# ubc-vision/DiffuseSG

Hardware: NVIDIA B200
Metric: sampled scene graphs/sec (higher is better)
Workload: dtype bf16

## Files before the change

diffusesg_b200/csrc/blockhead.cu:

```cuda
#include <cstdlib>

#include "common.cuh"
#include "kernels.h"

namespace dsg {
namespace {

constexpr int kHeadThreads = 19 * 32;
constexpr float kHeadLnEps = 1e-5f;

template <int C>
struct HeadCfg {
  static constexpr int N3 = 3 * C;
  static constexpr int KBN = C / 32;
  static constexpr int W_KB = C * 64;
  static constexpr int W_BYTES = 3 * KBN * W_KB;
  static constexpr int XB = C / 32;
  static constexpr int X_BYTES = XB * 16384;
  static constexpr int QB = C / 32;
  static constexpr int Q_BYTES = QB * 8192;
  static constexpr int CW = C / 4;
  static constexpr int PAR_FLOATS = N3 + 2 * C;
  static constexpr int PART_BYTES = 4 * 128 * 4;
  static constexpr int SMEM_BYTES = 1024 + W_BYTES + 2 * X_BYTES + 2 * Q_BYTES + PART_BYTES + PAR_FLOATS * 4 + 256;
  static constexpr int Y_COL = 3 * C;
  static_assert(C % 32 == 0 && CW % 8 == 0, "head: C must be a multiple of 32");
  static_assert(Y_COL + C / 2 <= 512 && SMEM_BYTES <= 227 * 1024, "head budget");
};

struct HeadParams {
  const float* film;
  int film_ld;
  int cond_uniform;
  int tokens_per_sample;
  const float* gamma;
  const float* beta;
  const float* bqkv;
  int M;
};

DSG_DEVICE uint64_t umma_desc_sw64_h(uint32_t smem_addr) {
  const uint64_t lo = ((smem_addr & 0x3FFFFu) >> 4) | (1ull << 16);
  const uint64_t hi = (512u >> 4) | (1u << 14) | (4u << 29);
  return lo | (hi << 32);
}
DSG_DEVICE void umma_bf16_ts_h(uint32_t tmem_d, uint32_t tmem_a, uint64_t b_desc, uint32_t idesc, uint32_t accumulate) {
  asm volatile(
      "{\n\t"
      ".reg .pred p;\n\t"
      "setp.ne.b32 p, %4, 0;\n\t"
      "tcgen05.mma.cta_group::1.kind::f16 [%0], [%1], %2, %3, p;\n\t"
      "}"
      ::"r"(tmem_d), "r"(tmem_a), "l"(b_desc), "r"(idesc), "r"(accumulate)
      : "memory");
}
DSG_DEVICE void tmem_ld_32x8_h(uint32_t taddr, uint32_t* r) {
  asm volatile("tcgen05.ld.sync.aligned.32x32b.x8.b32 {%0, %1, %2, %3, %4, %5, %6, %7}, [%8];"
               : "=r"(r[0]), "=r"(r[1]), "=r"(r[2]), "=r"(r[3]), "=r"(r[4]), "=r"(r[5]), "=r"(r[6]), "=r"(r[7])
               : "r"(taddr)
               : "memory");
}
DSG_DEVICE void tmem_st_32x4_h(uint32_t taddr, const uint32_t* r) {
  asm volatile("tcgen05.st.sync.aligned.32x32b.x4.b32 [%0], {%1, %2, %3, %4};"
               ::"r"(taddr), "r"(r[0]), "r"(r[1]), "r"(r[2]), "r"(r[3])
               : "memory");
}
DSG_DEVICE void tmem_st_wait_h() { asm volatile("tcgen05.wait::st.sync.aligned;" ::: "memory"); }
DSG_DEVICE void tma_store_2d_h(const CUtensorMap* map, const void* smem_src, int c_inner, int c_outer) {
  asm volatile("cp.async.bulk.tensor.2d.global.shared::cta.bulk_group [%0, {%2, %3}], [%1];"
               ::"l"(reinterpret_cast<uint64_t>(map)), "r"(smem_u32(smem_src)), "r"(c_inner), "r"(c_outer)
               : "memory");
}

template <int C>
__global__ void __launch_bounds__(kHeadThreads, 1)
block_head_kernel(const __grid_constant__ CUtensorMap tmXin, const __grid_constant__ CUtensorMap tmXout,
                  const __grid_constant__ CUtensorMap tmW, const __grid_constant__ CUtensorMap tmQ, const HeadParams p) {
  using G = HeadCfg<C>;
  extern __shared__ uint8_t smem_raw[];
  uint8_t* smem = smem_raw + ((1024u - (smem_u32(smem_raw) & 1023u)) & 1023u);
  uint8_t* sW = smem;
  uint8_t* sX = sW + G::W_BYTES;
  uint8_t* sXo = sX + G::X_BYTES;
  uint8_t* sQ = sXo + G::X_BYTES;
  float* sPart = reinterpret_cast<float*>(sQ + 2 * G::Q_BYTES);
  float* sBq = reinterpret_cast<float*>(reinterpret_cast<uint8_t*>(sPart) + G::PART_BYTES);
  float* sGam = sBq + G::N3;
  float* sBet = sGam + C;
  uint64_t* bars = reinterpret_cast<uint64_t*>(sBet + C);
  uint64_t* w_full = bars;
  uint64_t* xin_full = bars + 1;
  uint64_t* xin_free = bars + 2;
  uint64_t* xo_ready = bars + 3;
  uint64_t* xo_free = bars + 4;
  uint64_t* y_ready = bars + 5;
  uint64_t* acc_full = bars + 6;
  uint64_t* acc_empty = bars + 7;
  uint64_t* q_ready = bars + 8;
  uint64_t* q_free = bars + 10;
  uint32_t* tmem_slot = reinterpret_cast<uint32_t*>(bars + 12);

  const int warp = uniform_warp_id();
  const int lane = threadIdx.x & 31;
  constexpr int kLoadWarp = 16, kMmaWarp = 17, kStoreWarp = 18;
  const int num_tiles = (p.M + 127) / 128;
  const int my_tiles = (num_tiles > static_cast<int>(blockIdx.x)) ? (num_tiles - blockIdx.x + gridDim.x - 1) / gridDim.x : 0;

  if (warp == kLoadWarp && lane == 0) {
    tma_prefetch_desc(&tmXin);
    tma_prefetch_desc(&tmXout);
    tma_prefetch_desc(&tmW);
    tma_prefetch_desc(&tmQ);
    mbar_init(w_full, 1);
    mbar_init(xin_full, 1);
    mbar_init(xin_free, 16);
    mbar_init(xo_ready, 16);
    mbar_init(xo_free, 1);
    mbar_init(y_ready, 16);
    mbar_init(acc_full, 1);
    mbar_init(acc_empty, 16);
    for (int b = 0; b < 2; ++b) { mbar_init(&q_ready[b], 16); mbar_init(&q_free[b], 1); }
    fence_barrier_init();
  }
  if (warp == kMmaWarp) tmem_alloc<512>(tmem_slot);
  for (int i = threadIdx.x; i < G::N3; i += kHeadThreads) sBq[i] = p.bqkv[i];
  for (int i = threadIdx.x; i < C; i += kHeadThreads) { sGam[i] = p.gamma[i]; sBet[i] = p.beta[i]; }
  tcgen05_fence_before();
  __syncthreads();
  tcgen05_fence_after();
  const uint32_t tmem_base = uniform_u32(*tmem_slot);

  if (warp == kLoadWarp) {
    if (elect_one()) {
      mbar_expect_tx(w_full, G::W_BYTES);
      for (int part = 0; part < 3; ++part)
        for (int kb = 0; kb < G::KBN; ++kb)
          tma_load_2d(sW + (part * G::KBN + kb) * G::W_KB, &tmW, w_full, kb * 32, part * C);
      auto load_x = [&](int tl) {
        const int tile = blockIdx.x + tl * gridDim.x;
        mbar_expect_tx(xin_full, G::X_BYTES);
        for (int xb = 0; xb < G::XB; ++xb) tma_load_2d(sX + xb * 16384, &tmXin, xin_full, xb * 32, tile * 128);
      };
      auto prefetch_x = [&](int tl) {
        const int tile = blockIdx.x + tl * gridDim.x;
        for (int xb = 0; xb < G::XB; ++xb)
          asm volatile("cp.async.bulk.prefetch.tensor.2d.L2.global.tile [%0, {%1, %2}];"
                       ::"l"(reinterpret_cast<uint64_t>(&tmXin)), "r"(xb * 32), "r"(tile * 128) : "memory");
// ... 101 lines not shown
      asm volatile("bar.sync 1, 512;" ::: "memory");
      const float mean = ((sPart[r_t] + sPart[128 + r_t]) + (sPart[256 + r_t] + sPart[384 + r_t])) * (1.0f / C);
      float qq = 0.f;
#pragma unroll
      for (int i = 0; i < G::CW; i += 4) {
        float4& x = v[i >> 2];
        x.x -= mean; x.y -= mean; x.z -= mean; x.w -= mean;
        qq += (x.x * x.x + x.y * x.y) + (x.z * x.z + x.w * x.w);
      }
      asm volatile("bar.sync 2, 512;" ::: "memory");
      sPart[cg * 128 + r_t] = qq;
      asm volatile("bar.sync 1, 512;" ::: "memory");
      const float rstd =
          rsqrtf(((sPart[r_t] + sPart[128 + r_t]) + (sPart[256 + r_t] + sPart[384 + r_t])) * (1.0f / C) + kHeadLnEps);
      if (tl > 0) mbar_wait(acc_full, (tl - 1) & 1);
      tcgen05_fence_after();
#pragma unroll
      for (int i = 0; i < G::CW; i += 8) {
        const float4 g0 = *reinterpret_cast<const float4*>(&sGam[c0 + i]), g1 = *reinterpret_cast<const float4*>(&sGam[c0 + i + 4]);
        const float4 b0 = *reinterpret_cast<const float4*>(&sBet[c0 + i]), b1 = *reinterpret_cast<const float4*>(&sBet[c0 + i + 4]);
        const float4 xa = v[i >> 2], xb = v[(i >> 2) + 1];
        uint32_t pk[4];
        pk[0] = pack_bf16x2(fmaf(xa.x * rstd, g0.x, b0.x), fmaf(xa.y * rstd, g0.y, b0.y));
        pk[1] = pack_bf16x2(fmaf(xa.z * rstd, g0.z, b0.z), fmaf(xa.w * rstd, g0.w, b0.w));
        pk[2] = pack_bf16x2(fmaf(xb.x * rstd, g1.x, b1.x), fmaf(xb.y * rstd, g1.y, b1.y));
        pk[3] = pack_bf16x2(fmaf(xb.z * rstd, g1.z, b1.z), fmaf(xb.w * rstd, g1.w, b1.w));
        tmem_st_32x4_h(t_lane + G::Y_COL + ((c0 + i) >> 1), pk);
      }
      tmem_st_wait_h();
      tcgen05_fence_before();
      __syncwarp();
      if (lane == 0) mbar_arrive(y_ready);
    };

    int k = 0;
    auto phase_e = [&](int tl) {
      mbar_wait(acc_full, tl & 1);
      tcgen05_fence_after();
#pragma unroll 1
      for (int part = 0; part < 3; ++part, ++k) {
        const int b = k & 1;
        uint32_t v[G::CW];
#pragma unroll
        for (int i = 0; i < G::CW; i += 8) tmem_ld_32x8_h(t_lane + part * C + c0 + i, v + i);
        tmem_ld_wait();
        if (part == 2) {
          tcgen05_fence_before();
          __syncwarp();
          if (lane == 0) mbar_arrive(acc_empty);
        }
        if (k >= 2) mbar_wait(&q_free[b], ((k >> 1) - 1) & 1);
        uint8_t* buf = sQ + b * G::Q_BYTES;
#pragma unroll
        for (int i = 0; i < G::CW; i += 8) {
          const int c = c0 + i;
          const float4 ba = *reinterpret_cast<const float4*>(&sBq[part * C + c]);
          const float4 bb = *reinterpret_cast<const float4*>(&sBq[part * C + c + 4]);
          uint4 w;
          w.x = pack_bf16x2(__uint_as_float(v[i]) + ba.x, __uint_as_float(v[i + 1]) + ba.y);
          w.y = pack_bf16x2(__uint_as_float(v[i + 2]) + ba.z, __uint_as_float(v[i + 3]) + ba.w);
          w.z = pack_bf16x2(__uint_as_float(v[i + 4]) + bb.x, __uint_as_float(v[i + 5]) + bb.y);
          w.w = pack_bf16x2(__uint_as_float(v[i + 6]) + bb.z, __uint_as_float(v[i + 7]) + bb.w);
          *reinterpret_cast<uint4*>(buf + (c >> 5) * 8192 + r_t * 64 + (((((c & 31) >> 3)) ^ ((r_t >> 1) & 3)) << 4)) = w;
        }
        fence_proxy_async_smem();
        __syncwarp();
        if (lane == 0) mbar_arrive(&q_ready[b]);
      }
    };

    if (my_tiles > 0) phase_f(0);
    for (int tl = 0; tl < my_tiles; ++tl) {
      if (tl + 1 < my_tiles) phase_f(tl + 1);
      phase_e(tl);
    }
  }

  tcgen05_fence_before();
  __syncthreads();
  tcgen05_fence_after();
  if (warp == kMmaWarp) tmem_dealloc<512>(tmem_base);
}

}

bool block_head_supported(int C) { return C == 96; }

int launch_block_head(const CUtensorMap* tmXin, const CUtensorMap* tmXout, const CUtensorMap* tmW, const CUtensorMap* tmQ,
                      const float* film, int film_ld, int cond_uniform, int tokens_per_sample, const float* gamma,
                      const float* beta, const float* bqkv, long long rows, int C, cudaStream_t st) {
  DSG_REQUIRE(block_head_supported(C) && rows > 0 && rows < 2147483647LL, "block_head: C=%d rows=%lld", C, rows);
  using G = HeadCfg<96>;
  static PerDeviceOnce configured;
  if (configured.first()) {
    DSG_CUDA_CHECK(cudaFuncSetAttribute(block_head_kernel<96>, cudaFuncAttributeMaxDynamicSharedMemorySize, G::SMEM_BYTES));
  }
  const int sms = device_sm_count();
  HeadParams p{film, film_ld, cond_uniform, tokens_per_sample, gamma, beta, bqkv, static_cast<int>(rows)};
  const int tiles = (p.M + 127) / 128;
  block_head_kernel<96><<<tiles < sms ? tiles : sms, kHeadThreads, G::SMEM_BYTES, st>>>(*tmXin, *tmXout, *tmW, *tmQ, p);
  DSG_LAUNCH_CHECK();
  return DSG_OK;
}

}
```

diffusesg_b200/csrc/kernels.h:

```cpp
#pragma once

#include <cuda.h>
#include <cuda_bf16.h>
#include <cuda_runtime.h>
#include <stdint.h>

namespace dsg {

typedef __nv_bfloat16 bf16;

enum GemmEpi : int {
  EPI_BF16 = 0,
  EPI_GELU_BF16 = 1,
  EPI_RES_F32 = 2,
  EPI_F32 = 3,
  EPI_ADJ_HEAD = 4,
};

struct GemmParams {
  int M, N, K;
  const float* bias;
  const float* res;
  void* out;
  int ldo;
  int bn;
  int ksplit;
  int scale_rows;
  float row_scale;
  const float* w2t;
  const float* b2;
  int c_e;
  int n_img;
  const uint8_t* flags;
  const float* x_adj;
  const float* c_skip;
  const float* c_out;
  const int* perm;
  int side;
};

int make_tmap_bf16(CUtensorMap* map, const void* base, int64_t rows, int64_t cols, int box_rows);
int make_tmap_out(CUtensorMap* map, const void* base, int64_t rows, int64_t cols, int epi);

int launch_wgrad(const void* dy, const void* x, float* dw, long long tokens, int n_out, int x_cols, int out_cols, int ksplit,
                 int scale_rows, float row_scale, cudaStream_t st);

int gemm_block_n(int N);
int gemm_choose_bn(long long rows, int N, int K, int epi, bool pair);
bool gemm_use_pair(long long rows, int K, int epi);
int launch_gemm(const CUtensorMap* tmA, const CUtensorMap* tmW, const CUtensorMap* tmO, int epi, const GemmParams& p,
                cudaStream_t st, bool pair = false);

bool fused_mlp_supported(int C);
int fused_mlp_w1_box_rows(int C);
int launch_fused_mlp(const CUtensorMap* tmY, const CUtensorMap* tmW1, const CUtensorMap* tmW2, const CUtensorMap* tmX,
                     const float* b1, const float* b2, long long rows, int C, cudaStream_t st);

int make_tmap_2d(CUtensorMap* map, const void* base, int64_t rows, int64_t cols, int elem_bytes, int box_cols,
                 int box_rows);
bool block_tail_supported(int C);
int launch_block_tail(const CUtensorMap* tmAtt, const CUtensorMap* tmWp, const CUtensorMap* tmW1,
                      const CUtensorMap* tmW2, const CUtensorMap* tmX, const float* bp, const float* gamma,
                      const float* beta, const float* b1, const float* b2, float* x, long long rows, int C,
                      cudaStream_t st, const CUtensorMap* tmY = nullptr,
                      const float* gamma_f = nullptr, const float* beta_f = nullptr);

bool proj_ln_supported(int C);
int launch_proj_ln(const CUtensorMap* tmA, const CUtensorMap* tmW, const float* bias, const float* gamma, const float* beta,
                   float* x, bf16* y, long long rows, int C, cudaStream_t st);

bool block_head_supported(int C);
int launch_block_head(const CUtensorMap* tmXin, const CUtensorMap* tmXout, const CUtensorMap* tmW, const CUtensorMap* tmQ,
                      const float* film, int film_ld, int cond_uniform, int tokens_per_sample, const float* gamma,
                      const float* beta, const float* bqkv, long long rows, int C, cudaStream_t st);

int make_tmap_3d_bf16(CUtensorMap* map, const void* base, int64_t d0, int64_t d1, int64_t d2, int64_t s1, int64_t s2, int b0,
                      int b1, int b2);
bool window_attention_tc_supported(int batch, int res, int window, int shift, int heads);
int launch_window_attention_tc(const bf16* qkv, const float* bias, bf16* out, int batch, int res, int shift, int heads,
                               cudaStream_t st);
int launch_window_attention_tc_groups(const bf16* qkv, const float* bias, bf16* out, int n_groups, const int* counts,
                                      const int* res, const long long* tok_off, int heads, cudaStream_t st);
bool window_attention_quad_supported(int batch, int res, int window, int shift, int heads);
int launch_window_attention_quad(const bf16* qkv, const float* bias, bf16* out, int batch, int res, int window, int shift,
                                 int heads, cudaStream_t st);
int check_mask_canonical(const float* mask, int res, int window, int shift, cudaStream_t st, int* canonical);
bool window_attention_w16_supported(int batch, int res, int window, int shift, int heads);
int launch_window_attention_w16(const bf16* qkv, const float* bias, bf16* out, int batch, int res, int shift, int heads,
                                cudaStream_t st);
int check_bias_toeplitz(const float* bias, int heads, int window, cudaStream_t st, int* toeplitz);
enum { ATTN_MASK_CANONICAL = 1, ATTN_BIAS_TOEPLITZ = 2 };
int launch_window_attention(const bf16* qkv, const float* bias, const float* mask, bf16* out, int batch, int res,
                            int window, int shift, int heads, cudaStream_t st, int canonical = 0);

int launch_film_ln(const float* x_in, float* x_out, bf16* y, const float* film, int film_ld, int film_off,
                   int cond_uniform, const float* gamma, const float* beta, int batch, int tokens_per_sample,
                   int C, cudaStream_t st, const int* src_rows = nullptr);
int launch_ln(const float* x, bf16* y, const float* gamma, const float* beta, int64_t rows, int C, cudaStream_t st);
int launch_merge_ln(const float* x, bf16* y, const float* gamma, const float* beta, int batch, int res, int C,
                    cudaStream_t st);
int launch_concat_bf16(const float* x, const float* skip, bf16* y, int64_t rows, int C, cudaStream_t st,
                       const int* skip_rows = nullptr);
int launch_breakup_ln(const float* t, bf16* y, const float* g1, const float* b1, const float* g2, const float* b2,
                      int batch, int res, int D, cudaStream_t st, const int* tok0 = nullptr, const int* width = nullptr,
                      int sh = 0, const int* src_perm = nullptr);

int launch_cond(const float* noise_labels, long long label_stride, int n_cond, const float* w0, const float* b0, const float* w1,
                const float* b1, const float* w_film, const float* b_film, int film_total, float* emb0, float* emb1,
                float* emb, float* film, int embed, cudaStream_t st);

int launch_precond_coef(const float* sigmas, int sigma_stride, float* coef, int batch, cudaStream_t st);

int launch_node_proj(const float* node, const float* sc_node, const float* in_scale, const float* w_rc,
                     float* rc, int batch, int n, int c_n, int self_cond, int embed, cudaStream_t st);
int launch_patch_embed(const float* adj, const float* sc_adj, const float* in_scale, const uint8_t* flags,
                       const float* rc, const float* w_adj, const float* bias, const float* gamma,
                       const float* beta, const float* film, int film_ld, int film_off, int cond_uniform,
                       float* x0, int batch, int n, int c_e, int self_cond, int embed, cudaStream_t st,
                       const int* perm = nullptr, int side = 0);
int launch_node_head(const bf16* rep, const uint8_t* flags, const float* fold_t, const float* fold_b, const float* w1t,
                     const float* b1, const float* w2t, const float* b2, const float* x_node, const float* c_skip, const float* c_out,
                     float* out_node, int batch, int n, int c_n, int embed, cudaStream_t st, const int* tok0 = nullptr,
                     const int* width = nullptr, float* scratch = nullptr);


int launch_edm_pre_step(const float* adj, const float* node, const float* eps_adj, const float* eps_node,
                        const uint8_t* flags, float noise_coef, float* adj_hat, float* node_hat, int batch,
                        int c_e, int n, int c_n, cudaStream_t st);
int launch_edm_pre_step_philox(const float* adj, const float* node, const uint8_t* flags, float noise_coef,
                               unsigned long long seed, unsigned long long offset_adj, int grid_adj,
                               unsigned long long offset_node, int grid_node, const void* dev_params, float* adj_hat,
                               float* node_hat, int batch, int c_e, int n, int c_n, cudaStream_t st);
int launch_edm_post_step(const float* adj_hat, const float* node_hat, const float* d1_adj, const float* d1_node,
                         const float* d2_adj, const float* d2_node, const uint8_t* flags, float inv_t_hat,
                         float h, float inv_t_prime, const void* dev_params, float* adj_next, float* node_next, int batch,
                         int c_e, int n, int c_n, cudaStream_t st);
int launch_edm_step_advance(const void* table, void* cur, int* counter, cudaStream_t st);
int launch_edm_final_decode(const float* adj_hat, const float* node_hat, const float* d1_adj, const float* d1_node,
                            const uint8_t* flags, float inv_t_hat, float h, const void* dev_params, float* adj_next,
                            float* node_next, int32_t* adj_cls, int32_t* node_cls, float* bbox, int num_adj_type,
                            int num_node_type, int batch, int c_e, int n, int c_n, cudaStream_t st);
int launch_mask_scale(const float* adj, const float* node, const uint8_t* flags, float scale, float* adj_out,
                      float* node_out, int batch, int c_e, int n, int c_n, cudaStream_t st);

int launch_decode(const float* adj, const float* node, const uint8_t* flags, int32_t* adj_cls, int32_t* node_cls,
                  float* bbox, int num_adj_type, int num_node_type, int batch, int c_e, int n, int c_n, cudaStream_t st);

int launch_train_noise(const float* y_adj, const float* y_node, const float* e_adj, const float* e_node,
                       const float* sigmas, const uint8_t* flags, float* x_adj, float* n_adj, float* x_node,
                       float* n_node, int batch, int c_e, int n, int c_n, cudaStream_t st);
int launch_loss_sums(const float* d_adj, const float* y_adj, const float* d_node, const float* y_node,
                     const float* weights, const uint8_t* flags, float* s_adj, float* s_node, int batch, int c_e, int n,
                     int c_n, cudaStream_t st);
int launch_loss_sums_backward(const float* d_adj, const float* y_adj, const float* d_node, const float* y_node,
                              const float* weights, const uint8_t* flags, const float* g_adj, const float* g_node,
                              float* gd_adj, float* gd_node, int batch, int c_e, int n, int c_n, cudaStream_t st);

// ... 12 lines not shown
```

diffusesg_b200/csrc/model.cu:

```cuda
#include <cstdarg>
#include <cstdio>
#include <cstdlib>
#include <cstring>
#include <map>
#include <string>
#include <tuple>
#include <vector>

#include "../../include/dsg_b200.h"
#include "common.cuh"
#include "kernels.h"

namespace dsg {

static thread_local char g_err[1024] = "";
static unsigned long long g_launches = 0;
static int g_stop_after = -1;

void set_last_error(const char* fmt, ...) {
  va_list ap;
  va_start(ap, fmt);
  vsnprintf(g_err, sizeof(g_err), fmt, ap);
  va_end(ap);
}
// ... 442 lines not shown
  for (int s = 0; s + 1 < m->nl; ++s) w.skip.push_back(static_cast<float*>(take((full >> (s + 1)) * 4)));
  w.coef = static_cast<float*>(take(static_cast<size_t>(4) * batch * 4));
  w.emb0 = static_cast<float*>(take(static_cast<size_t>(n_cond) * m->E * 4));
  w.emb1 = static_cast<float*>(take(static_cast<size_t>(n_cond) * 512 * 4));
  w.emb = static_cast<float*>(take(static_cast<size_t>(n_cond) * 512 * 4));
  w.film = static_cast<float*>(take(static_cast<size_t>(n_cond) * m->film_total * 4));
  w.rc = static_cast<float*>(take(static_cast<size_t>(batch) * m->N * 2 * m->E * 4));
  w.bytes = cur;
  return w;
}

int gemm(dsg_model* m, const bf16* A, long long rows, const Weight& W, int epi, const float* bias, const float* res,
         void* out, cudaStream_t st, const GemmParams* extra = nullptr) {
  DSG_REQUIRE(rows > 0 && rows < 2147483647LL, "gemm: %lld rows", rows);
  auto key = std::make_tuple(static_cast<const void*>(A), rows, W.K);
  auto it = m->a_maps.find(key);
  if (it == m->a_maps.end()) {
    CUtensorMap tm;
    int rc = make_tmap_bf16(&tm, A, rows, W.K, 128);
    if (rc) return rc;
    if (m->a_maps.size() > 4096) m->a_maps.clear();
    it = m->a_maps.emplace(key, tm).first;
  }
  const CUtensorMap* tmo = &it->second;
  if (epi != EPI_ADJ_HEAD) {
    auto okey = std::make_tuple(static_cast<const void*>(out), rows, -(W.N * 8 + epi));
    auto ot = m->a_maps.find(okey);
    if (ot == m->a_maps.end()) {
      CUtensorMap tm;
      int rc = make_tmap_out(&tm, out, rows, W.N, epi);
      if (rc) return rc;
      ot = m->a_maps.emplace(okey, tm).first;
    }
    tmo = &ot->second;
  }
  GemmParams p;
  if (extra) p = *extra; else memset(&p, 0, sizeof(p));
  p.M = static_cast<int>(rows); p.N = W.N; p.K = W.K;
  p.bias = bias; p.res = res; p.out = out; p.ldo = W.N;
  const double mn = static_cast<double>(rows) * W.N;
  const double out_bytes = epi == EPI_ADJ_HEAD ? static_cast<double>(rows) * (extra ? extra->c_e : 0) * 4
                                               : mn * ((epi == EPI_BF16 || epi == EPI_GELU_BF16) ? 2 : 4);
  char label[56];
  snprintf(label, sizeof(label), "gemm_n%d_k%d_epi%d", W.N, W.K, epi);
  ProfScope ps(g_prof_pass, PC_GEMM, 2.0 * mn * W.K,
               static_cast<double>(rows) * W.K * 2 + static_cast<double>(W.N) * W.K * 2 + out_bytes +
                   (epi == EPI_RES_F32 ? mn * 4 : 0), st, label, rows, W.K);
  const bool pair = gemm_use_pair(rows, W.K, epi);
  p.bn = gemm_choose_bn(rows, W.N, W.K, epi, pair);
  if (p.bn == 256) return launch_gemm(&it->second, pair ? &W.tmap256_half : &W.tmap256, tmo, epi, p, st, pair);
  return launch_gemm(&it->second, pair ? &W.tmap_half : &W.tmap, tmo, epi, p, st, pair);
}

#define DSG_TRY(expr)        \
  do {                       \
    int _rc = (expr);        \
    if (_rc) return _rc;     \
  } while (0)

#define DSG_TRY_P(cls, flops, bytes, expr)                                    \
  do {                                                                        \
    ProfScope _ps(g_prof_pass, cls, flops, bytes, st, #expr);                 \
    int _rc = (expr);                                                         \
    if (_rc) return _rc;                                                      \
  } while (0)

int run_block(dsg_model* m, const Block& b, const Workspace& w, const float* x_in, const Layout& lay, const int* x_in_rows,
              int cond_uniform, cudaStream_t st, bool fuse_final_ln, bool* fused_final_ln) {
  const int C = b.dim;
  const int L = b.res * b.res;
  const long long rows = lay.tokens(b.stage);
  const std::string& p = b.prefix;
  const double rc = static_cast<double>(rows) * C;
  auto tmap = [&](const void* ptr, int key, auto make) -> const CUtensorMap* {
    auto k = std::make_tuple(ptr, rows, key);
    auto it = m->a_maps.find(k);
    if (it == m->a_maps.end()) {
      CUtensorMap tm;
      if (make(&tm)) return nullptr;
      it = m->a_maps.emplace(k, tm).first;
    }
    return &it->second;
  };
  DSG_REQUIRE(x_in_rows == nullptr || (x_in != w.X && !block_head_supported(C)), "run_block: layout-changing input at C = %d", C);
  if (m->use_head && block_head_supported(C)) {
    const CUtensorMap* ti = tmap(x_in, -(C * 8 + EPI_RES_F32), [&](CUtensorMap* t) { return make_tmap_out(t, x_in, rows, C, EPI_RES_F32); });
    const CUtensorMap* to = tmap(w.X, -(C * 8 + EPI_RES_F32), [&](CUtensorMap* t) { return make_tmap_out(t, w.X, rows, C, EPI_RES_F32); });
    const CUtensorMap* tq = tmap(w.QKV, -(3 * C * 8 + EPI_BF16), [&](CUtensorMap* t) { return make_tmap_out(t, w.QKV, rows, 3 * C, EPI_BF16); });
    if (ti == nullptr || to == nullptr || tq == nullptr) return DSG_ERR_CUDA;
    DSG_TRY_P(PC_MLP, 6.0 * rc * C, rc * 14,
              launch_block_head(ti, to, &b.head_w, tq, w.film + b.film_off, m->film_total, cond_uniform, L,
                                m->f32(p + ".norm1.weight"), m->f32(p + ".norm1.bias"), m->at<float>(b.qkv_bias_off), rows,
                                C, st));
  } else {
    const int per_sample = cond_uniform ? static_cast<int>(rows) : L;
    DSG_TRY_P(PC_ROW, 0, rc * 10, launch_film_ln(x_in, w.X, w.Y, w.film, m->film_total, b.film_off, cond_uniform,
                                                 m->f32(p + ".norm1.weight"), m->f32(p + ".norm1.bias"),
                                                 static_cast<int>(rows / per_sample), per_sample, C, st, x_in_rows));
    DSG_TRY(gemm(m, w.Y, rows, b.qkv, EPI_BF16, m->at<float>(b.qkv_bias_off), nullptr, w.QKV, st));
  }
  const float* mask = b.shift > 0 ? m->f32(p + ".attn_mask") : nullptr;
  if (!lay.dense() && b.window == 8 && lay.K <= 4) {
    int res_k[4];
    long long tok_k[4];
    for (int k = 0; k < lay.K; ++k) { res_k[k] = lay.side[k] >> b.stage; tok_k[k] = lay.at(k, b.stage); }
    DSG_TRY_P(PC_ATTN, 4.0 * rc * b.window * b.window, rc * 8,
              launch_window_attention_tc_groups(w.QKV, m->at<float>(b.attn_bias_off), w.ATT, lay.K, lay.count, res_k, tok_k, b.heads, st));
  } else {
    for (int k = 0; k < lay.K; ++k) {
      const long long t0 = lay.at(k, b.stage), tk = lay.at(k + 1, b.stage) - t0;
      DSG_TRY_P(PC_ATTN, 4.0 * tk * C * b.window * b.window, static_cast<double>(tk) * C * 8,
                launch_window_attention(w.QKV + t0 * 3 * C, m->at<float>(b.attn_bias_off), mask, w.ATT + t0 * C, lay.count[k],
                                        lay.side[k] >> b.stage, b.window, b.shift, b.heads, st, b.mask_canonical));
    }
  }
  if (m->use_tail && block_tail_supported(C)) {
    const CUtensorMap* ta = tmap(w.ATT, 100000 + C, [&](CUtensorMap* t) { return make_tmap_2d(t, w.ATT, rows, C, 2, 32, 128); });
    const CUtensorMap* tx = tmap(w.X, -(C * 8 + EPI_RES_F32), [&](CUtensorMap* t) { return make_tmap_out(t, w.X, rows, C, EPI_RES_F32); });
    if (ta == nullptr || tx == nullptr) return DSG_ERR_CUDA;
    const CUtensorMap* ty = nullptr;
    if (fuse_final_ln) {
      ty = tmap(w.Y, -(C * 8 + EPI_BF16), [&](CUtensorMap* t) { return make_tmap_out(t, w.Y, rows, C, EPI_BF16); });
      if (ty == nullptr) return DSG_ERR_CUDA;
      if (fused_final_ln) *fused_final_ln = true;
    }
    DSG_TRY_P(PC_MLP, 18.0 * rc * C, rc * (fuse_final_ln ? 8 : 10),
              launch_block_tail(ta, &b.tail_wp, &b.tail_w1, &b.mlp_w2, tx, m->f32(p + ".attn.proj.bias"),
                                m->f32(p + ".norm2.weight"), m->f32(p + ".norm2.bias"), m->f32(p + ".mlp.fc1.bias"),
                                m->f32(p + ".mlp.fc2.bias"), w.X, rows, C, st, ty,
                                fuse_final_ln ? m->f32("norm.weight") : nullptr,
                                fuse_final_ln ? m->f32("norm.bias") : nullptr));
    return DSG_OK;
  }
  if (C == 384) {
    const CUtensorMap* ta = tmap(w.ATT, C, [&](CUtensorMap* t) { return make_tmap_bf16(t, w.ATT, rows, C, 128); });
    if (ta == nullptr) return DSG_ERR_CUDA;
    DSG_TRY_P(PC_MLP, 2.0 * rc * C, rc * 12,
              launch_proj_ln(ta, &b.proj.tmap, m->f32(p + ".attn.proj.bias"), m->f32(p + ".norm2.weight"),
                             m->f32(p + ".norm2.bias"), w.X, w.Y, rows, C, st));
  } else {
    DSG_TRY(gemm(m, w.ATT, rows, b.proj, EPI_RES_F32, m->f32(p + ".attn.proj.bias"), w.X, w.X, st));
    DSG_TRY_P(PC_ROW, 0, rc * 6, launch_ln(w.X, w.Y, m->f32(p + ".norm2.weight"), m->f32(p + ".norm2.bias"), rows, C, st));
  }
  if (m->use_fused_mlp && fused_mlp_supported(C)) {
    const CUtensorMap* ty = tmap(w.Y, C, [&](CUtensorMap* t) { return make_tmap_bf16(t, w.Y, rows, C, 128); });
    const CUtensorMap* tx = tmap(w.X, -(C * 8 + EPI_RES_F32), [&](CUtensorMap* t) { return make_tmap_out(t, w.X, rows, C, EPI_RES_F32); });
    if (ty == nullptr || tx == nullptr) return DSG_ERR_CUDA;
    DSG_TRY_P(PC_MLP, 16.0 * rc * C, rc * 10,
              launch_fused_mlp(ty, &b.mlp_w1, &b.mlp_w2, tx, m->f32(p + ".mlp.fc1.bias"), m->f32(p + ".mlp.fc2.bias"), rows,
                               C, st));
    return DSG_OK;
  }
  DSG_TRY(gemm(m, w.Y, rows, b.fc1, EPI_GELU_BF16, m->f32(p + ".mlp.fc1.bias"), nullptr, w.H, st));
  DSG_TRY(gemm(m, w.H, rows, b.fc2, EPI_RES_F32, m->f32(p + ".mlp.fc2.bias"), w.X, w.X, st));
  return DSG_OK;
}

}

extern "C" {

int dsg_abi_version(void) { return DSG_ABI_VERSION; }
void dsg_debug_set_smem_poison(unsigned pattern, int enable) {
  g_smem_poison = pattern;
  g_smem_poison_on = enable != 0;
}
const char* dsg_last_error(void) { return g_err; }
uint64_t dsg_launch_count(void) { return __atomic_load_n(&g_launches, __ATOMIC_RELAXED); }

int dsg_model_create(const dsg_config* cfg, dsg_model** out) {
  DSG_REQUIRE(cfg != nullptr && out != nullptr, "dsg_model_create: null argument");
  dsg_model* m = new dsg_model();
  m->cfg = *cfg;
  const char* no_fuse = getenv("DSG_NO_FUSED_MLP");
// ... 3 lines not shown
  const char* no_head = getenv("DSG_NO_HEAD");
  m->use_head = !(no_head != nullptr && no_head[0] == '1');
  const int rc = build(m);
  if (rc) { delete m; return rc; }
  *out = m;
  return DSG_OK;
}

void dsg_model_destroy(dsg_model* m) { delete m; }

size_t dsg_model_arena_bytes(const dsg_model* m) { return m ? m->arena_bytes : 0; }

int dsg_model_bind_arena(dsg_model* m, void* arena, size_t bytes) {
  DSG_REQUIRE(m != nullptr && arena != nullptr, "bind_arena: null argument");
  if (bytes < m->arena_bytes || (reinterpret_cast<uintptr_t>(arena) & (kAlign - 1)) != 0) {
    set_last_error("bind_arena: need %zu bytes aligned to %zu, got %zu at %p", m->arena_bytes, kAlign, bytes, arena);
    return DSG_ERR_WORKSPACE;
  }
  m->arena = static_cast<uint8_t*>(arena);
  m->finalized = false;
  for (TensorSpec& t : m->tensors) t.loaded = false;
  return DSG_OK;
}

int dsg_model_num_tensors(const dsg_model* m) { return m ? static_cast<int>(m->tensors.size()) : 0; }

int dsg_model_tensor_info(const dsg_model* m, int i, const char** key, int64_t* numel, int32_t* dtype) {
  DSG_REQUIRE(m != nullptr && i >= 0 && i < static_cast<int>(m->tensors.size()), "tensor_info: index %d", i);
  if (key) *key = m->tensors[i].key.c_str();
  if (numel) *numel = m->tensors[i].numel;
  if (dtype) *dtype = m->tensors[i].dtype;
  return DSG_OK;
}

int dsg_model_set_tensor(dsg_model* m, const char* key, const void* src, int64_t bytes, int src_is_host,
                         dsg_stream_t stream) {
  DSG_REQUIRE(m != nullptr && key != nullptr && src != nullptr, "set_tensor: null argument");
  if (m->arena == nullptr) { set_last_error("set_tensor: no arena bound"); return DSG_ERR_STATE; }
  auto it = m->index.find(key);
  if (it == m->index.end()) { set_last_error("set_tensor: unknown key '%s'", key); return DSG_ERR_UNKNOWN_KEY; }
  TensorSpec& t = m->tensors[it->second];
  DSG_REQUIRE(static_cast<size_t>(bytes) == t.bytes(), "set_tensor: '%s' expects %zu bytes, got %lld", key, t.bytes(),
              static_cast<long long>(bytes));
  DSG_CUDA_CHECK(cudaMemcpyAsync(m->arena + t.offset, src, t.bytes(),
                                 src_is_host ? cudaMemcpyHostToDevice : cudaMemcpyDeviceToDevice,
                                 static_cast<cudaStream_t>(stream)));
  t.loaded = true;
  m->finalized = false;
  return DSG_OK;
}

int dsg_model_tensor_differs(const dsg_model* m, const char* key, const void* src, int64_t bytes, int32_t* flag,
                             dsg_stream_t stream) {
  DSG_REQUIRE(m != nullptr && key != nullptr && src != nullptr && flag != nullptr, "tensor_differs: null argument");
  if (m->arena == nullptr) { set_last_error("tensor_differs: no arena bound"); return DSG_ERR_STATE; }
  auto it = m->index.find(key);
  if (it == m->index.end()) { set_last_error("tensor_differs: unknown key '%s'", key); return DSG_ERR_UNKNOWN_KEY; }
  const TensorSpec& t = m->tensors[it->second];
  DSG_REQUIRE(static_cast<size_t>(bytes) == t.bytes() && (reinterpret_cast<uintptr_t>(src) & 3) == 0,
              "tensor_differs: '%s' expects %zu bytes (4-byte aligned), got %lld", key, t.bytes(), static_cast<long long>(bytes));
  return launch_compare_words(m->arena + t.offset, src, static_cast<int64_t>(t.bytes() / 4), flag,
                              static_cast<cudaStream_t>(stream));
}

int dsg_model_finalize(dsg_model* m, dsg_stream_t stream) {
  DSG_REQUIRE(m != nullptr, "finalize: null model");
  if (m->arena == nullptr) { set_last_error("finalize: no arena bound"); return DSG_ERR_STATE; }
  for (const TensorSpec& t : m->tensors)
    if (!t.loaded) { set_last_error("finalize: tensor '%s' was never set", t.key.c_str()); return DSG_ERR_STATE; }
  cudaStream_t st = static_cast<cudaStream_t>(stream);
  const float qscale = 0.17677669529663687f;
  for (Block& b : m->blocks) {
    const int C = b.dim, T = b.window * b.window;
    const std::string& p = b.prefix;
    DSG_TRY(pack_weight(m, b.qkv, p + ".attn.qkv.weight", st, static_cast<int64_t>(C) * C, qscale));
    DSG_TRY(launch_scale_copy(m->f32(p + ".attn.qkv.bias"), m->at<float>(b.qkv_bias_off), 3 * C, C, qscale, st));
    DSG_TRY(pack_weight(m, b.proj, p + ".attn.proj.weight", st));
    DSG_TRY(pack_weight(m, b.fc1, p + ".mlp.fc1.weight", st));
    DSG_TRY(pack_weight(m, b.fc2, p + ".mlp.fc2.weight", st));
    if (fused_mlp_supported(C)) {
      DSG_TRY(make_tmap_bf16(&b.mlp_w1, m->arena + b.fc1.offset, 4 * C, C, fused_mlp_w1_box_rows(C)));
      DSG_TRY(make_tmap_bf16(&b.mlp_w2, m->arena + b.fc2.offset, C, 4 * C, C));
    }
    if (block_head_supported(C)) DSG_TRY(make_tmap_2d(&b.head_w, m->arena + b.qkv.offset, 3 * C, C, 2, 32, C));
    if (block_tail_supported(C)) {
      DSG_TRY(make_tmap_2d(&b.tail_wp, m->arena + b.proj.offset, C, C, 2, 32, C));
      DSG_TRY(make_tmap_2d(&b.tail_w1, m->arena + b.fc1.offset, 4 * C, C, 2, 32, 128));
    }
    const TensorSpec& idx = m->tensors[m->index[p + ".attn.relative_position_index"]];
    DSG_TRY(launch_bias_expand(m->f32(p + ".attn.relative_position_bias_table"),
                               reinterpret_cast<const int64_t*>(m->arena + idx.offset), m->at<float>(b.attn_bias_off), T,
                               b.heads, (2 * b.window - 1) * (2 * b.window - 1), st));
    b.mask_canonical = 0;
    const bool w16 = window_attention_w16_supported(1, b.res, b.window, b.shift, b.heads);
    if (b.shift > 0 && (w16 || window_attention_quad_supported(1, b.res, b.window, b.shift, b.heads))) {
      int ok = 0;
      DSG_TRY(check_mask_canonical(m->f32(p + ".attn_mask"), b.res, b.window, b.shift, st, &ok));
      if (ok) b.mask_canonical |= ATTN_MASK_CANONICAL;
    }
    if (w16) {
      int ok = 0;
      DSG_TRY(check_bias_toeplitz(m->at<float>(b.attn_bias_off), b.heads, b.window, st, &ok));
      if (ok) b.mask_canonical |= ATTN_BIAS_TOEPLITZ;
    }
  }
  for (Merge& g : m->merges) DSG_TRY(pack_weight(m, g.reduction, g.prefix + ".reduction.weight", st));
  for (Breakup& u : m->breakups) {
    DSG_TRY(pack_weight(m, u.pre, u.prefix + ".pre_linear.weight", st));
    DSG_TRY(pack_weight(m, u.post, u.prefix + ".post_linear.weight", st));
  }
  const int E = m->E;
  const float* wp = m->f32("patch_embed.proj.weight");
  DSG_TRY(launch_transpose(wp, m->at<float>(m->w_adj_off), E, m->cin, 0, m->planes_adj, E, st));
  DSG_TRY(launch_transpose(wp, m->at<float>(m->w_rc_off), E, m->cin, m->planes_adj, m->planes_node, E, st));
  DSG_TRY(launch_transpose(wp, m->at<float>(m->w_rc_off) + static_cast<size_t>(m->planes_node) * E, E, m->cin,
                           m->planes_adj + m->planes_node, m->planes_node, E, st));
  float* t1 = m->at<float>(m->fold_t1_off);
  float* ff = m->at<float>(m->fold_f_off);
  float* tv = m->at<float>(m->fold_tv_off);
  DSG_TRY(launch_small_mm(m->f32("read_out.1.weight"), m->f32("read_out.0.weight"), t1, E, 1, st));
  DSG_TRY(launch_small_mm(m->f32("read_out.2.weight"), t1, ff, E, 0, st));
  DSG_TRY(launch_small_mv(m->f32("read_out.1.weight"), m->f32("read_out.0.bias"), m->f32("read_out.1.bias"), tv, E, st));
  DSG_TRY(launch_small_mv(m->f32("read_out.2.weight"), tv, m->f32("read_out.2.bias"), m->at<float>(m->fold_b_off), E, st));
  DSG_TRY(launch_small_mm(m->f32("readout_adj_mlp.fc1.weight"), ff, t1, E, 0, st));
  DSG_TRY(launch_pack_bf16(t1, m->at<bf16>(m->adj_fc1.offset), static_cast<int64_t>(E) * E, 0, 1.f, st));
  DSG_TRY(make_tmap_bf16(&m->adj_fc1.tmap, m->arena + m->adj_fc1.offset, E, E, gemm_block_n(E)));
  DSG_TRY(launch_small_mv(m->f32("readout_adj_mlp.fc1.weight"), m->at<float>(m->fold_b_off),
                          m->f32("readout_adj_mlp.fc1.bias"), m->at<float>(m->adj_b1_off), E, st));
  DSG_TRY(launch_transpose(ff, m->at<float>(m->fold_ft_off), E, E, 0, E, E, st));
  DSG_CUDA_CHECK(cudaMemsetAsync(m->at<float>(m->adj_w2t_off), 0, static_cast<size_t>(E) * 8 * 4, st));
  DSG_CUDA_CHECK(cudaMemsetAsync(m->at<float>(m->adj_b2_off), 0, 8 * 4, st));
  DSG_TRY(launch_transpose(m->f32("readout_adj_mlp.fc2.weight"), m->at<float>(m->adj_w2t_off), m->cfg.c_e, E, 0, E, 8, st));
  DSG_CUDA_CHECK(cudaMemcpyAsync(m->at<float>(m->adj_b2_off), m->f32("readout_adj_mlp.fc2.bias"), m->cfg.c_e * 4,
                                 cudaMemcpyDeviceToDevice, st));
  DSG_TRY(launch_transpose(m->f32("readout_node_mlp.fc1.weight"), m->at<float>(m->node_w1t_off), E, E, 0, E, E, st));
  DSG_TRY(launch_transpose(m->f32("readout_node_mlp.fc2.weight"), m->at<float>(m->node_w2t_off), m->cfg.c_n, E, 0, E,
                           m->cfg.c_n, st));
  m->finalized = true;
  return DSG_OK;
}

int dsg_model_skip_info(const dsg_model* m, int32_t* stages, int32_t* granule) {
  DSG_REQUIRE(m != nullptr && stages != nullptr && granule != nullptr, "skip_info: null argument");
  *stages = m->skip_stages;
  *granule = m->skip_granule;
  return DSG_OK;
}

int dsg_model_skip_info2(const dsg_model* m, int32_t* granule2) {
  DSG_REQUIRE(m != nullptr && granule2 != nullptr, "skip_info2: null argument");
  *granule2 = m->skip2_granule;
  return DSG_OK;
}

size_t dsg_workspace_bytes(const dsg_model* m, int batch, int n_cond) {
  if (m == nullptr || batch <= 0 || n_cond <= 0) return 0;
  return carve(m, batch, n_cond, nullptr).bytes;
}

int dsg_denoiser_forward(dsg_model* m, const dsg_forward_args* a, dsg_stream_t stream) {
  DSG_REQUIRE(m != nullptr && a != nullptr, "forward: null argument");
  DSG_REQUIRE(a->struct_size == sizeof(dsg_forward_args), "forward: dsg_forward_args size %u, library expects %zu",
              a->struct_size, sizeof(dsg_forward_args));
  if (!m->finalized) { set_last_error("forward: dsg_model_finalize has not been called since the last weight update"); return DSG_ERR_STATE; }
  DSG_REQUIRE(a->batch > 0 && (a->n_cond == 1 || a->n_cond == a->batch), "forward: batch %d n_cond %d", a->batch, a->n_cond);
  DSG_REQUIRE(a->mode == 0 || a->mode == 1, "forward: mode %d", a->mode);
  DSG_REQUIRE(a->adj && a->node && a->flags && a->noise && a->out_adj && a->out_node, "forward: null tensor");
// ... 409 lines not shown
```

Measured before the change: 66.64.

## Add streaming fused FiLM+LayerNorm+QKV head kernel for C=192 and 384

Extends the fused block head (FiLM modulation, SiLU, LayerNorm, QKV GEMM with bias) to channel widths 192 and 384 via a new warp-specialized kernel. Normalized activations are staged in shared memory, copied into tensor memory, and consumed by tcgen05 MMAs while weight chunks stream through a multi-stage TMA pipeline. Output tiles go out through TMA stores. It also supports gathered input rows, replacing the separate film_ln kernel plus GEMM path at these widths and saving the intermediate Y round trip. The cost is much more complex synchronization, plus per-tile weight reloads that may pressure L2.

```diff
diff --git a/diffusesg_b200/csrc/blockhead.cu b/diffusesg_b200/csrc/blockhead.cu
--- a/diffusesg_b200/csrc/blockhead.cu
+++ b/diffusesg_b200/csrc/blockhead.cu
@@ -63,6 +63,11 @@
 DSG_DEVICE void tmem_st_32x4_h(uint32_t taddr, const uint32_t* r) {
   asm volatile("tcgen05.st.sync.aligned.32x32b.x4.b32 [%0], {%1, %2, %3, %4};"
                ::"r"(taddr), "r"(r[0]), "r"(r[1]), "r"(r[2]), "r"(r[3])
+               : "memory");
+}
+DSG_DEVICE void tmem_st_32x8_h(uint32_t taddr, const uint32_t* r) {
+  asm volatile("tcgen05.st.sync.aligned.32x32b.x8.b32 [%0], {%1, %2, %3, %4, %5, %6, %7, %8};"
+               ::"r"(taddr), "r"(r[0]), "r"(r[1]), "r"(r[2]), "r"(r[3]), "r"(r[4]), "r"(r[5]), "r"(r[6]), "r"(r[7])
                : "memory");
 }
 DSG_DEVICE void tmem_st_wait_h() { asm volatile("tcgen05.wait::st.sync.aligned;" ::: "memory"); }
@@ -330,14 +335,334 @@
   if (warp == kMmaWarp) tmem_dealloc<512>(tmem_base);
 }
 
-}
-
-bool block_head_supported(int C) { return C == 96; }
+constexpr int kStreamThreads = 19 * 32;
+
+template <int C>
+struct StreamCfg {
+  static constexpr int N = (C == 384) ? 96 : 192;
+  static constexpr int NCH = 3 * C / N;
+  static constexpr int NACC = (C == 384) ? 3 : 2;
+  static constexpr int KB = C / 64;
+  static constexpr int STAGE_BYTES = N * 128;
+  static constexpr int kStages = (C == 384) ? 8 : 5;
+  static constexpr int Y_BYTES = KB * 16384;
+  static constexpr int kQBufs = 4;
+  static constexpr int SMEM_BYTES = 1024 + Y_BYTES + kStages * STAGE_BYTES + kQBufs * 8192 + 512;
+  static constexpr int LPR = C / 12;
+  static constexpr int RPW = 32 / LPR;
+  static constexpr int kSlots = 2;
+  static constexpr int RI = kSlots * RPW;
+  static constexpr int ITERS = 16 / RI;
+  static constexpr int Y_COL = NACC * N;
+  static_assert(C % 192 == 0 && 16 % RI == 0 && N % 32 == 0, "stream head: C = 192 or 384");
+  static_assert(Y_COL + C / 2 <= 512 && SMEM_BYTES <= 227 * 1024, "stream head budget");
+};
+
+struct StreamParams {
+  const float* x_in;
+  float* x_out;
+  const int* x_in_rows;
+  const float* film;
+  int film_ld;
+  int cond_uniform;
+  int tokens_per_sample;
+  const float* gamma;
+  const float* beta;
+  const float* bqkv;
+  int M;
+};
+
+DSG_DEVICE uint32_t sw128_off_h(int r, int k) {
+  return static_cast<uint32_t>((k >> 6) * 16384 + r * 128 + ((((k & 63) >> 3) ^ (r & 7)) << 4));
+}
+
+template <int C>
+__global__ void __launch_bounds__(kStreamThreads, 1)
+block_head_stream_kernel(const __grid_constant__ CUtensorMap tmW, const __grid_constant__ CUtensorMap tmQ,
+                         const StreamParams p) {
+  using G = StreamCfg<C>;
+  extern __shared__ uint8_t smem_raw[];
+  uint8_t* smem = smem_raw + ((1024u - (smem_u32(smem_raw) & 1023u)) & 1023u);
+  uint8_t* sY = smem;
+  uint8_t* sW = sY + G::Y_BYTES;
+  uint8_t* sQ = sW + G::kStages * G::STAGE_BYTES;
+  uint64_t* bars = reinterpret_cast<uint64_t*>(sQ + G::kQBufs * 8192);
+  uint64_t* w_full = bars;
+  uint64_t* w_empty = w_full + G::kStages;
+  uint64_t* acc_full = w_empty + G::kStages;
+  uint64_t* acc_empty = acc_full + G::NACC;
+  uint64_t* q_ready = acc_empty + G::NACC;
+  uint64_t* q_free = q_ready + G::kQBufs;
+  uint64_t* sy_full = q_free + G::kQBufs;
+  uint64_t* sy_free = sy_full + 1;
+  uint64_t* y_full = sy_full + 2;
+  uint32_t* tmem_slot = reinterpret_cast<uint32_t*>(sy_full + 3);
+
+  const int warp = uniform_warp_id();
+  const int lane = threadIdx.x & 31;
+  constexpr int kLoadWarp = 16, kMmaWarp = 17, kStoreWarp = 18;
+  const int num_tiles = (p.M + 127) / 128;
+  const int my_tiles = (num_tiles > static_cast<int>(blockIdx.x)) ? (num_tiles - blockIdx.x + gridDim.x - 1) / gridDim.x : 0;
+
+  if (warp == kLoadWarp && lane == 0) {
+    tma_prefetch_desc(&tmW);
+    tma_prefetch_desc(&tmQ);
+    for (int s = 0; s < G::kStages; ++s) { mbar_init(&w_full[s], 1); mbar_init(&w_empty[s], 1); }
+    for (int b = 0; b < G::NACC; ++b) { mbar_init(&acc_full[b], 1); mbar_init(&acc_empty[b], 8); }
+    for (int b = 0; b < G::kQBufs; ++b) { mbar_init(&q_ready[b], 8); mbar_init(&q_free[b], 1); }
+    mbar_init(sy_full, 8);
+    mbar_init(sy_free, 8);
+    mbar_init(y_full, 8);
+    fence_barrier_init();
+  }
+  if (warp == kMmaWarp) tmem_alloc<512>(tmem_slot);
+  tcgen05_fence_before();
+  __syncthreads();
+  tcgen05_fence_after();
+  const uint32_t tmem_base = uniform_u32(*tmem_slot);
+
+  if (warp == kLoadWarp) {
+    if (elect_one()) {
+      int s = 0;
+      uint32_t ph = 0;
+      for (int t = 0; t < my_tiles; ++t)
+        for (int j = 0; j < G::NCH; ++j)
+          for (int kb = 0; kb < G::KB; ++kb) {
+            mbar_wait(&w_empty[s], ph ^ 1);
+            mbar_expect_tx(&w_full[s], G::STAGE_BYTES);
+            tma_load_2d(sW + s * G::STAGE_BYTES, &tmW, &w_full[s], kb * 64, j * G::N);
+            if (++s == G::kStages) { s = 0; ph ^= 1; }
+          }
+    }
+  } else if (warp == kMmaWarp) {
+    constexpr uint32_t idesc = umma_idesc_bf16(G::N);
+    int s = 0, g = 0;
+    uint32_t ph = 0;
+    for (int t = 0; t < my_tiles; ++t) {
+      mbar_wait(y_full, t & 1);
+      for (int j = 0; j < G::NCH; ++j, ++g) {
+        const int b = g % G::NACC;
+        mbar_wait(&acc_empty[b], ((g / G::NACC) & 1) ^ 1);
+        tcgen05_fence_after();
+        for (int kb = 0; kb < G::KB; ++kb) {
+          mbar_wait(&w_full[s], ph);
+          tcgen05_fence_after();
+          if (elect_one()) {
+            const uint64_t db = umma_desc_sw128(smem_u32(sW + s * G::STAGE_BYTES));
+            for (int k = 0; k < 4; ++k)
+              umma_bf16_ts_h(tmem_base + b * G::N, tmem_base + G::Y_COL + (kb * 4 + k) * 8, db + 2 * k, idesc, (kb | k) != 0);
+            umma_commit(&w_empty[s]);
+          }
+          __syncwarp();
+          if (++s == G::kStages) { s = 0; ph ^= 1; }
+        }
+        if (elect_one()) umma_commit(&acc_full[b]);
+        __syncwarp();
+      }
+    }
+  } else if (warp == kStoreWarp) {
+    if (elect_one()) {
+      uint64_t* prev_free = nullptr;
+      int kq = 0;
+      for (int t = 0; t < my_tiles; ++t) {
+        const int tile = blockIdx.x + t * gridDim.x;
+        for (int j = 0; j < G::NCH; ++j)
+          for (int bx = 0; bx < G::N / 32; ++bx, ++kq) {
+            const int sb = kq % G::kQBufs;
+            mbar_wait(&q_ready[sb], (kq / G::kQBufs) & 1);
+            tma_store_2d_h(&tmQ, sQ + sb * 8192, j * G::N + bx * 32, tile * 128);
+            asm volatile("cp.async.bulk.commit_group;" ::: "memory");
+            asm volatile("cp.async.bulk.wait_group.read 1;" ::: "memory");
+            if (prev_free != nullptr) mbar_arrive(prev_free);
+            prev_free = &q_free[sb];
+          }
+      }
+      asm volatile("cp.async.bulk.wait_group 0;" ::: "memory");
+    }
+  } else if (warp < 8) {
+    const int sr = lane / G::LPR, ll = lane % G::LPR;
+    auto prefetch_rows = [&](int tl) {
+      constexpr int kLines = C / 32;
+      const long long row0 = static_cast<long long>(blockIdx.x + tl * gridDim.x) * 128 + warp * 16;
+#pragma unroll
+      for (int k = 0; k < kLines / 2; ++k) {
+        const int idx = lane + 32 * k;
+        const long long row = row0 + idx / kLines;
+        if (row < p.M) {
+          const long long src = p.x_in_rows != nullptr ? static_cast<long long>(p.x_in_rows[row]) : row;
+          asm volatile("prefetch.global.L2 [%0];" ::"l"(p.x_in + src * C + (idx % kLines) * 32) : "memory");
+        }
+      }
+    };
+    if (my_tiles > 0) prefetch_rows(0);
+    for (int t = 0; t < my_tiles; ++t) {
+      const int tile = blockIdx.x + t * gridDim.x;
+      if (t + 1 < my_tiles) prefetch_rows(t + 1);
+#pragma unroll 1
+      for (int it = 0; it < G::ITERS; ++it) {
+        float4 v[G::kSlots][3];
+        int rows[G::kSlots];
+#pragma unroll
+        for (int s = 0; s < G::kSlots; ++s) {
+          const int rt = warp * 16 + it * G::RI + s * G::RPW + sr;
+          const long long row = static_cast<long long>(tile) * 128 + rt;
+          rows[s] = static_cast<int>(row < p.M ? row : p.M - 1);
+          const long long src = p.x_in_rows != nullptr ? static_cast<long long>(p.x_in_rows[rows[s]]) : rows[s];
+          const float* xr = p.x_in + src * C + 4 * ll;
+#pragma unroll
+          for (int i = 0; i < 3; ++i) v[s][i] = *reinterpret_cast<const float4*>(xr + 4 * G::LPR * i);
+        }
+        if (it == 0) mbar_wait(sy_free, (t & 1) ^ 1);
+#pragma unroll
+        for (int s = 0; s < G::kSlots; ++s) {
+          const int rt = warp * 16 + it * G::RI + s * G::RPW + sr;
+          const bool valid = static_cast<long long>(tile) * 128 + rt < p.M;
+          const float* fs = p.film + static_cast<size_t>(p.cond_uniform ? 0 : rows[s] / p.tokens_per_sample) * p.film_ld;
+          float sum = 0.f;
+#pragma unroll
+          for (int i = 0; i < 3; ++i) {
+            const int c = 4 * ll + 4 * G::LPR * i;
+            const float4 sc = __ldg(reinterpret_cast<const float4*>(fs + c));
+            const float4 sh = __ldg(reinterpret_cast<const float4*>(fs + C + c));
+            float4& x = v[s][i];
+            x.x = silu_f(fmaf(x.x, sc.x + 1.f, sh.x)); x.y = silu_f(fmaf(x.y, sc.y + 1.f, sh.y));
+            x.z = silu_f(fmaf(x.z, sc.z + 1.f, sh.z)); x.w = silu_f(fmaf(x.w, sc.w + 1.f, sh.w));
+            if (valid) *reinterpret_cast<float4*>(p.x_out + static_cast<long long>(rows[s]) * C + c) = x;
+            sum += (x.x + x.y) + (x.z + x.w);
+          }
+#pragma unroll
+          for (int o = G::LPR / 2; o > 0; o >>= 1) sum += __shfl_xor_sync(0xffffffffu, sum, o);
+          const float mean = sum * (1.0f / C);
+          float qq = 0.f;
+#pragma unroll
+          for (int i = 0; i < 3; ++i) {
+            float4& x = v[s][i];
+            x.x -= mean; x.y -= mean; x.z -= mean; x.w -= mean;
+            qq += (x.x * x.x + x.y * x.y) + (x.z * x.z + x.w * x.w);
+          }
+#pragma unroll
+          for (int o = G::LPR / 2; o > 0; o >>= 1) qq += __shfl_xor_sync(0xffffffffu, qq, o);
+          const float rstd = rsqrtf(qq * (1.0f / C) + kHeadLnEps);
+#pragma unroll
+          for (int i = 0; i < 3; ++i) {
+            const int c = 4 * ll + 4 * G::LPR * i;
+            const float4 gg = __ldg(reinterpret_cast<const float4*>(p.gamma + c));
+            const float4 bb = __ldg(reinterpret_cast<const float4*>(p.beta + c));
+            const float4 x = v[s][i];
+            uint2 y;
+            y.x = pack_bf16x2(fmaf(x.x * rstd, gg.x, bb.x), fmaf(x.y * rstd, gg.y, bb.y));
+            y.y = pack_bf16x2(fmaf(x.z * rstd, gg.z, bb.z), fmaf(x.w * rstd, gg.w, bb.w));
+            *reinterpret_cast<uint2*>(sY + sw128_off_h(rt, c) + (c & 4) * 2) = y;
+          }
+        }
+      }
+      __syncwarp();
+      if (lane == 0) mbar_arrive(sy_full);
+    }
+  } else {
+    const int q = warp & 3;
+    const int h = (warp - 8) >> 2;
+    const int r_t = q * 32 + lane;
+    const uint32_t t_lane = tmem_base + (static_cast<uint32_t>(q * 32) << 16);
+
+    auto copy_y = [&](int t) {
+      mbar_wait(sy_full, t & 1);
+#pragma unroll 4
+      for (int c = h * (C / 2); c < (h + 1) * (C / 2); c += 16) {
+        const uint4 a = *reinterpret_cast<const uint4*>(sY + sw128_off_h(r_t, c));
+        const uint4 b = *reinterpret_cast<const uint4*>(sY + sw128_off_h(r_t, c + 8));
+        const uint32_t w[8] = {a.x, a.y, a.z, a.w, b.x, b.y, b.z, b.w};
+        tmem_st_32x8_h(t_lane + G::Y_COL + c / 2, w);
+      }
+      tmem_st_wait_h();
+      tcgen05_fence_before();
+      __syncwarp();
+      if (lane == 0) {
+        mbar_arrive(sy_free);
+        mbar_arrive(y_full);
+      }
+    };
+
+    if (my_tiles > 0) copy_y(0);
+    int g = 0, kq = 0;
+    for (int t = 0; t < my_tiles; ++t) {
+#pragma unroll 1
+      for (int j = 0; j < G::NCH; ++j, ++g) {
+        const int b = g % G::NACC;
+        mbar_wait(&acc_full[b], (g / G::NACC) & 1);
+        tcgen05_fence_after();
+        if (j == G::NCH - 1 && t + 1 < my_tiles) copy_y(t + 1);
+#pragma unroll 1
+        for (int bx = 0; bx < G::N / 32; ++bx, ++kq) {
+          uint32_t v[16];
+          tmem_ld_32x16(t_lane + b * G::N + bx * 32 + h * 16, v);
+          tmem_ld_wait();
+          if (bx == G::N / 32 - 1) {
+            tcgen05_fence_before();
+            __syncwarp();
+            if (lane == 0) mbar_arrive(&acc_empty[b]);
+          }
+          const int sb = kq % G::kQBufs;
+          mbar_wait(&q_free[sb], ((kq / G::kQBufs) & 1) ^ 1);
+          const float* bias = p.bqkv + j * G::N + bx * 32 + h * 16;
+          uint32_t w[8];
+#pragma unroll
+          for (int i = 0; i < 16; i += 4) {
+            const float4 bb = __ldg(reinterpret_cast<const float4*>(bias + i));
+            w[i >> 1] = pack_bf16x2(__uint_as_float(v[i]) + bb.x, __uint_as_float(v[i + 1]) + bb.y);
+            w[(i >> 1) + 1] = pack_bf16x2(__uint_as_float(v[i + 2]) + bb.z, __uint_as_float(v[i + 3]) + bb.w);
+          }
+          uint8_t* rowp = sQ + sb * 8192 + r_t * 64;
+#pragma unroll
+          for (int u = 0; u < 2; ++u)
+            *reinterpret_cast<uint4*>(rowp + (((h * 2 + u) ^ ((r_t >> 1) & 3)) << 4)) =
+                make_uint4(w[4 * u], w[4 * u + 1], w[4 * u + 2], w[4 * u + 3]);
+          fence_proxy_async_smem();
+          __syncwarp();
+          if (lane == 0) mbar_arrive(&q_ready[sb]);
+        }
+      }
+    }
+  }
+
+  tcgen05_fence_before();
+  __syncthreads();
+  tcgen05_fence_after();
+  if (warp == kMmaWarp) tmem_dealloc<512>(tmem_base);
+}
+
+template <int C>
+int launch_stream(const CUtensorMap* tmW, const CUtensorMap* tmQ, const StreamParams& p, cudaStream_t st) {
+  using G = StreamCfg<C>;
+  static PerDeviceOnce configured;
+  if (configured.first()) {
+    DSG_CUDA_CHECK(cudaFuncSetAttribute(block_head_stream_kernel<C>, cudaFuncAttributeMaxDynamicSharedMemorySize,
+                                        G::SMEM_BYTES));
+  }
+  const int sms = device_sm_count();
+  const int tiles = (p.M + 127) / 128;
+  block_head_stream_kernel<C><<<tiles < sms ? tiles : sms, kStreamThreads, G::SMEM_BYTES, st>>>(*tmW, *tmQ, p);
+  DSG_LAUNCH_CHECK();
+  return DSG_OK;
+}
+
+}
+
+bool block_head_supported(int C) { return C == 96 || C == 192 || C == 384; }
 
 int launch_block_head(const CUtensorMap* tmXin, const CUtensorMap* tmXout, const CUtensorMap* tmW, const CUtensorMap* tmQ,
-                      const float* film, int film_ld, int cond_uniform, int tokens_per_sample, const float* gamma,
-                      const float* beta, const float* bqkv, long long rows, int C, cudaStream_t st) {
+                      const float* x_in, float* x_out, const int* x_in_rows, const float* film, int film_ld,
+                      int cond_uniform, int tokens_per_sample, const float* gamma, const float* beta, const float* bqkv,
+                      long long rows, int C, cudaStream_t st) {
   DSG_REQUIRE(block_head_supported(C) && rows > 0 && rows < 2147483647LL, "block_head: C=%d rows=%lld", C, rows);
+  DSG_REQUIRE(x_in_rows == nullptr || (C != 96 && x_in != x_out),
+              "block_head: a gathering launch needs C = 192 or 384 and cannot run in place (C=%d)", C);
+  if (C != 96) {
+    StreamParams p{x_in, x_out, x_in_rows, film, film_ld, cond_uniform, tokens_per_sample, gamma, beta, bqkv,
+                   static_cast<int>(rows)};
+    return C == 384 ? launch_stream<384>(tmW, tmQ, p, st) : launch_stream<192>(tmW, tmQ, p, st);
+  }
+  DSG_REQUIRE(tmXin != nullptr && tmXout != nullptr, "block_head: C = 96 needs the x tensor maps");
   using G = HeadCfg<96>;
   static PerDeviceOnce configured;
   if (configured.first()) {
diff --git a/diffusesg_b200/csrc/kernels.h b/diffusesg_b200/csrc/kernels.h
--- a/diffusesg_b200/csrc/kernels.h
+++ b/diffusesg_b200/csrc/kernels.h
@@ -71,8 +71,9 @@
 
 bool block_head_supported(int C);
 int launch_block_head(const CUtensorMap* tmXin, const CUtensorMap* tmXout, const CUtensorMap* tmW, const CUtensorMap* tmQ,
-                      const float* film, int film_ld, int cond_uniform, int tokens_per_sample, const float* gamma,
-                      const float* beta, const float* bqkv, long long rows, int C, cudaStream_t st);
+                      const float* x_in, float* x_out, const int* x_in_rows, const float* film, int film_ld,
+                      int cond_uniform, int tokens_per_sample, const float* gamma, const float* beta, const float* bqkv,
+                      long long rows, int C, cudaStream_t st);
 
 int make_tmap_3d_bf16(CUtensorMap* map, const void* base, int64_t d0, int64_t d1, int64_t d2, int64_t s1, int64_t s2, int b0,
                       int b1, int b2);
diff --git a/diffusesg_b200/csrc/model.cu b/diffusesg_b200/csrc/model.cu
--- a/diffusesg_b200/csrc/model.cu
+++ b/diffusesg_b200/csrc/model.cu
@@ -548,14 +548,19 @@
     }
     return &it->second;
   };
-  DSG_REQUIRE(x_in_rows == nullptr || (x_in != w.X && !block_head_supported(C)), "run_block: layout-changing input at C = %d", C);
+  DSG_REQUIRE(x_in_rows == nullptr || x_in != w.X, "run_block: layout-changing input in place at C = %d", C);
   if (m->use_head && block_head_supported(C)) {
-    const CUtensorMap* ti = tmap(x_in, -(C * 8 + EPI_RES_F32), [&](CUtensorMap* t) { return make_tmap_out(t, x_in, rows, C, EPI_RES_F32); });
-    const CUtensorMap* to = tmap(w.X, -(C * 8 + EPI_RES_F32), [&](CUtensorMap* t) { return make_tmap_out(t, w.X, rows, C, EPI_RES_F32); });
+    const CUtensorMap *ti = nullptr, *to = nullptr;
+    if (C == 96) {
+      ti = tmap(x_in, -(C * 8 + EPI_RES_F32), [&](CUtensorMap* t) { return make_tmap_out(t, x_in, rows, C, EPI_RES_F32); });
+      to = tmap(w.X, -(C * 8 + EPI_RES_F32), [&](CUtensorMap* t) { return make_tmap_out(t, w.X, rows, C, EPI_RES_F32); });
+      if (ti == nullptr || to == nullptr) return DSG_ERR_CUDA;
+    }
     const CUtensorMap* tq = tmap(w.QKV, -(3 * C * 8 + EPI_BF16), [&](CUtensorMap* t) { return make_tmap_out(t, w.QKV, rows, 3 * C, EPI_BF16); });
-    if (ti == nullptr || to == nullptr || tq == nullptr) return DSG_ERR_CUDA;
+    if (tq == nullptr) return DSG_ERR_CUDA;
+    const CUtensorMap* tw = C == 96 ? &b.head_w : C == 384 ? &b.qkv.tmap_half : &b.qkv.tmap;
     DSG_TRY_P(PC_MLP, 6.0 * rc * C, rc * 14,
-              launch_block_head(ti, to, &b.head_w, tq, w.film + b.film_off, m->film_total, cond_uniform, L,
+              launch_block_head(ti, to, tw, tq, x_in, w.X, x_in_rows, w.film + b.film_off, m->film_total, cond_uniform, L,
                                 m->f32(p + ".norm1.weight"), m->f32(p + ".norm1.bias"), m->at<float>(b.qkv_bias_off), rows,
                                 C, st));
   } else {
@@ -725,7 +730,7 @@
       DSG_TRY(make_tmap_bf16(&b.mlp_w1, m->arena + b.fc1.offset, 4 * C, C, fused_mlp_w1_box_rows(C)));
       DSG_TRY(make_tmap_bf16(&b.mlp_w2, m->arena + b.fc2.offset, C, 4 * C, C));
     }
-    if (block_head_supported(C)) DSG_TRY(make_tmap_2d(&b.head_w, m->arena + b.qkv.offset, 3 * C, C, 2, 32, C));
+    if (C == 96) DSG_TRY(make_tmap_2d(&b.head_w, m->arena + b.qkv.offset, 3 * C, C, 2, 32, C));
     if (block_tail_supported(C)) {
       DSG_TRY(make_tmap_2d(&b.tail_wp, m->arena + b.proj.offset, C, C, 2, 32, C));
       DSG_TRY(make_tmap_2d(&b.tail_w1, m->arena + b.fc1.offset, 4 * C, C, 2, 32, 128));
```

Result: slower. 65.86, median of 6 (-1.2%).
